# zhoupengwei/tloam

Hardware: AMD Instinct MI355X
Metric: gauss_newton_iters_per_sec (higher is better)
Workload: dtype f64

## Files before the change

tloam_amd/csrc/tl_api.hip:

```cpp
#include "tl_ctx.hpp"

using namespace tl;

extern "C" {

int tloam_abi_version(void) { return TLOAM_ABI_VERSION; }

const char* tloam_status_string(int s) {
  switch (s) {
    case TLOAM_OK: return "ok";
    case TLOAM_E_INVALID: return "invalid argument";
    case TLOAM_E_TOO_FEW_POINTS: return "fewer than 10 points in a feature cloud";
    case TLOAM_E_BAD_POSE: return "predicted pose is not a rigid transform";
    case TLOAM_E_HIP: return "HIP error / no gfx950 device";
    case TLOAM_E_RCCL: return "RCCL error";
    case TLOAM_E_NOT_READY: return "call sequence violated";
    case TLOAM_E_WEIGHT_RANGE: return "GNC weight outside [0,1]";
    default: return "unknown status";
  }
}

void tloam_default_config(tloam_tls_config* c) {
  if (!c) return;
  memset(c, 0, sizeof(*c));
  c->k_corr = 10;
  c->factor_num = 4;
  c->edge_dist_thres = 1.0;
  c->edge_dir_thres = 0.85;
  c->edge_maxnum = 1200;
  c->sphere_dist_thres = 0.5;
  c->sphere_maxnum = 200;
  c->planar_dist_thres = 0.5;
  c->planar_maxnum = 2500;
  c->ground_dist_thres = 0.5;
  c->ground_maxnum = 2000;
  c->max_iterations = 4;
  c->cost_threshold = 5e-9;
  c->gnc_factor = 11.8;
  c->noise_bound = 0.01;
  c->fitness_thres = 0.02;
}

int tloam_create(const tloam_tls_config* cfg, int device_id, tloam_ctx** out) {
  if (!cfg || !out) return TLOAM_E_INVALID;
  *out = nullptr;
  (void)setenv("HIP_FORCE_DEV_KERNARG", "1", 0);
  int ndev = 0;
  if (hipGetDeviceCount(&ndev) != hipSuccess || ndev <= 0 || device_id < 0 || device_id >= ndev) return TLOAM_E_HIP;
  if (hipSetDevice(device_id) != hipSuccess) return TLOAM_E_HIP;
  tloam_ctx* c = new (std::nothrow) tloam_ctx();
  if (!c) return TLOAM_E_INVALID;
  c->cfg = *cfg;
  c->device = device_id;
  if (const char* e = getenv("TLOAM_DEBUG_MAX_SWEEPS")) c->dbg_max_sweeps = atoi(e);
  c->dbg_no_build_reuse = getenv("TLOAM_NO_BUILD_REUSE") != nullptr;
  c->dbg_no_eval_reuse = getenv("TLOAM_NO_EVAL_REUSE") != nullptr;
  c->no_device_loop = getenv("TLOAM_NO_DEVICE_LOOP") != nullptr;
  c->no_persistent_solve = getenv("TLOAM_NO_PERSISTENT_SOLVE") != nullptr;
  c->no_grid_ahead = getenv("TLOAM_NO_GRID_AHEAD") != nullptr;
  c->no_direct_set = getenv("TLOAM_NO_DIRECT_SET") != nullptr;
  c->no_qbin_ride = getenv("TLOAM_NO_QBIN_RIDE") != nullptr;
  if (const char* e = getenv("TLOAM_DEBUG_FAIL_HANDOVER")) c->dbg_fail_handover = atoi(e);
  {
    int cus = 0;
    if (hipDeviceGetAttribute(&cus, hipDeviceAttributeMultiprocessorCount, device_id) != hipSuccess) cus = 0;
    c->device_cus = cus;
  }
  c->fused_large = getenv("TLOAM_FUSED_LARGE") != nullptr;
  if (const char* e = getenv("TLOAM_PLANNED_SWEEPS")) c->dbg_planned_sweeps = atoi(e);
  memset(&c->stats, 0, sizeof(c->stats));
  if (hipStreamCreateWithFlags(&c->stream, hipStreamNonBlocking) != hipSuccess ||
      hipHostMalloc((void**)&c->h_state, sizeof(GnState) * kMirrorSlots, hipHostMallocMapped | hipHostMallocCoherent) != hipSuccess ||
      hipHostMalloc((void**)&c->h_small, sizeof(double) * 4096, hipHostMallocDefault) != hipSuccess) {
    delete c;
    return TLOAM_E_HIP;
  }
  memset(c->h_state, 0, sizeof(GnState) * kMirrorSlots);
  {
    constexpr size_t kBoxBytes = sizeof(double) * ((size_t)kKinds * 64 * 6 + 8);
    const unsigned flags = hipHostMallocMapped | hipHostMallocCoherent;
    if (hipHostMalloc((void**)&c->h_mirror, sizeof(MirrorSlot) * kMirrorSlots, flags) != hipSuccess ||
        ((uintptr_t)c->h_mirror & 63u) != 0 || hipHostGetDevicePointer((void**)&c->h_mirror_dev, c->h_mirror, 0) != hipSuccess ||
        hipHostMalloc((void**)&c->h_bbox, kBoxBytes, flags) != hipSuccess ||
        hipHostGetDevicePointer((void**)&c->h_bbox_dev, c->h_bbox, 0) != hipSuccess ||
        hipHostMalloc((void**)&c->h_fault, sizeof(unsigned) * kFaultWords, flags) != hipSuccess ||
        hipHostGetDevicePointer((void**)&c->h_fault_dev, c->h_fault, 0) != hipSuccess) {
      (void)hipGetLastError();
      tloam_destroy(c);
      return TLOAM_E_HIP;
    }
    memset(c->h_mirror, 0, sizeof(MirrorSlot) * kMirrorSlots);
    memset(c->h_bbox, 0, kBoxBytes);
    memset(c->h_fault, 0, sizeof(unsigned) * kFaultWords);
  }
  if (ensure_common(c) != TLOAM_OK) { tloam_destroy(c); return TLOAM_E_HIP; }
  (void)hipMemsetAsync(c->state.p, 0, sizeof(GnState), c->stream);
  (void)hipMemsetAsync(c->seg_n.p, 0, 8 * sizeof(int), c->stream);
  (void)hipStreamSynchronize(c->stream);
  *out = c;
  return TLOAM_OK;
}

void tloam_destroy(tloam_ctx* c) {
  if (!c) return;
  (void)hipSetDevice(c->device);
  if (c->stream) (void)hipStreamSynchronize(c->stream);
  tlh::comm_release(c);
  c->scan1p_q.release(); c->k3_ticket.release(); c->k3_span.release(); c->iter_span.release(); c->state_scratch.release(); c->blk_cnt.release(); c->row_of_pos.release(); c->fin_tickets.release(); c->fin_rows.release(); c->flagb.release();
  for (auto& e : c->ev_pool) (void)hipEventDestroy(e);
  if (c->frame_selected >= 0) { exchange_clouds(c, *c->frame_store[c->frame_selected]); c->frame_selected = -1; }
  for (int k = 0; k < kKinds; ++k) {
    KindData& K = c->kd[k];
    K.src_aos.release(); K.tgt_aos.release(); K.tx.release(); K.ty.release(); K.tz.release();
    K.c_idx.release(); K.c_buf.release();
// ... 103 lines not shown
```

tloam_amd/csrc/tl_api_match.hip:

```cpp
#include <atomic>
#include <chrono>

#include "tl_ctx.hpp"

using namespace tl;

namespace {
int sync_stream(tloam_ctx* c) {
  HIPC(c, hipStreamSynchronize(c->stream));
  return TLOAM_OK;
}
}

namespace tlh {
int reserve_seg(tloam_ctx* c, int k, size_t n) {
  KindData& K = c->kd[k];
  const size_t cap = round_up(std::max<size_t>(n, 1), kChunk) + kChunk;
  HIPC(c, K.c_idx.reserve(cap));
  if (cap > K.c_stride) {
    const size_t stride = std::max(cap, K.c_stride + K.c_stride / 2);
    HIPC(c, K.c_buf.reserve(stride * kSegStreams));
    K.c_stride = stride;
  }
  K.c_cap = cap - kChunk;
// ... 385 lines not shown
constexpr int kMaxOuterFast = kMirrorSlots;

void outer_params(const tloam_ctx* c, BuildParams* bp, GridView grids[kKinds]) {
  for (int k = 0; k < kKinds; ++k) {
    bp->radius[k] = kind_radius(c->cfg, k);
    bp->maxnum[k] = kind_maxnum(c->cfg, k);
    bp->active[k] = kind_active(c->cfg, k);
    grids[k] = c->kd[k].gv;
  }
  bp->edge_dir_thres = c->cfg.edge_dir_thres;
}
int outer_reserve(tloam_ctx* c, const GridView grids[kKinds]) { return tlh::reserve_query_sort(c, grids); }
}
extern "C++" {
namespace tlh {
int reserve_query_sort(tloam_ctx* c, const GridView grids[kKinds]) {
  const size_t n_slots = (size_t)c->sv.slot_off[kKinds];
  const size_t ntiles = (size_t)build_tile_count(grids, c->sv.slot_off);
  const size_t nt_res = (ntiles + 1 > c->tile_cnt.cap || ntiles + 1 > c->tile_scan.cap) ? 2 * ntiles + 64 : ntiles;
  {
    const size_t before = c->tile_cnt.cap;
    HIPC(c, c->tile_cnt.reserve(nt_res + 1));
    if (c->tile_cnt.cap != before)
      HIPC(c, hipMemsetAsync(c->tile_cnt.p, 0, c->tile_cnt.cap * sizeof(unsigned long long), c->stream));
  }
  HIPC(c, c->tile_scan.reserve(nt_res + 1));
  HIPC(c, c->tile_fill.reserve(std::max<size_t>((size_t)nt_res, (size_t)n_slots + 1))  ); HIPC(c, c->tile_of_slot.reserve(n_slots + 1));
  HIPC(c, c->qrec.reserve(n_slots + 1));
  HIPC(c, c->scan_tmp.reserve(scan_tmp_elems(std::max(nt_res + 1, n_slots + 1))));
  c->scan1p_q_use = !c->no_scan_1p && scan_1p_applies(ntiles + 1, c->device_cus);
  if (c->scan1p_q_use) {
    const size_t before = c->scan1p_q.cap;
    HIPC(c, c->scan1p_q.reserve(scan_1p_ctl_elems(nt_res + 1)));
    if (c->scan1p_q.cap != before) HIPC(c, hipMemsetAsync(c->scan1p_q.p, 0, c->scan1p_q.cap * sizeof(unsigned long long), c->stream));
  }
  return TLOAM_OK;
}
}
}
namespace {
bool prepare_small_path(const tloam_ctx* c) { return one_rank(c) && prepare_small_fits(c->sv); }
bool self_prepare_path(const tloam_ctx* c) { return c->sv.flagb != nullptr && prepare_small_path(c) && solve_small_path(c); }
int enqueue_build(tloam_ctx* c, const BuildParams& bp, const GridView grids[kKinds], bool rebin, const int* gate,
                  const int* refresh_gate = nullptr, bool prepare_in_solve = false, const FinishLargeArgs* ride = nullptr, int iter = 0) {
  const size_t n_slots = (size_t)c->sv.slot_off[kKinds];
  const DirectSet ds{c->direct ? 1 : 0, rebin ? 1 : 0, (ride && !rebin) ? 0 : 1, c->direct ? direct_blk_cnt(c, iter) : nullptr,
                     c->tile_of_slot.p, c->tile_scan.p, c->direct ? c->row_of_pos.p : nullptr};
  if (ride && !rebin) {
    const size_t ntiles = (size_t)build_tile_count(grids, c->sv.slot_off);
    launch_build_finish_large(c->sv, grids, bp, c->state.p, c->tile_scan.p + ntiles, c->qrec.p, *ride, c->stream, c->direct ? &ds : nullptr);
  } else {
    launch_build(c->sv, grids, bp, c->state.p, c->tile_of_slot.p, c->tile_cnt.p, c->tile_scan.p, c->tile_fill.p,
                 c->qrec.p, c->scan_tmp.p, rebin, c->stream, gate, c->scan1p_q_use ? c->scan1p_q.p : nullptr, c->h_fault_dev + kFaultScan1p,
                 c->direct ? &c->cv : nullptr, c->direct ? &ds : nullptr, rebin && c->qbin_rode);
    if (rebin) c->qbin_rode = false;
  }
  if (c->direct) return TLOAM_OK;
  if (prepare_in_solve) return TLOAM_OK;
  if (prepare_small_path(c)) {
    launch_prepare_small(c->sv, c->cv, bp, c->seg_n.p, c->state.p, gate, refresh_gate, c->stream);
    return TLOAM_OK;
  }
  if (one_rank(c)) {
    const int tiles = scan_tiles_only(c->flags.p, c->scan.p, n_slots + 1, c->scan_tmp.p, c->stream, gate);
    if (tiles > 0) {
      launch_compact(c->sv, c->cv, bp, c->seg_n.p, nullptr, 0, 1, c->state.p, c->stream, gate, refresh_gate, c->scan_tmp.p, tiles);
      return TLOAM_OK;
    }
  }
  launch_exclusive_scan_u64(c->flags.p, c->scan.p, n_slots + 1, c->scan_tmp.p, c->stream, gate);
  const double* rank_counts = nullptr;
  if (exchanging(c)) {
    launch_rank_counts(c->sv, c->rank_counts.p, c->rank, c->nranks, c->stream);
    const int rc = allreduce(c, c->rank_counts.p, c->nranks * kKinds);
    if (rc != TLOAM_OK) return rc;
    rank_counts = c->rank_counts.p;
  }
  if (exchanging(c)) HIPC(c, hipMemsetAsync(c->seg_n.p, 0, kKinds * sizeof(int), c->stream));
  launch_compact(c->sv, c->cv, bp, c->seg_n.p, rank_counts, c->rank, c->nranks, c->state.p, c->stream, gate);
  if (refresh_gate) launch_refresh(c->sv, c->cv, c->stream, refresh_gate);
  return TLOAM_OK;
}
int planned_sweeps_for(tloam_ctx* c, int iter) {
  if ((int)c->planned_sweeps.size() < 3 * (iter + 1)) c->planned_sweeps.resize(3 * ((size_t)iter + 1), 0);
  const int* hist = &c->planned_sweeps[3 * (size_t)iter];
  int planned = hist[0] == 0 ? kSolveSweeps
                             : std::min(std::max(std::max(hist[0], hist[1]), std::max(hist[2], 1)), kSolveSweeps);
  if (solve_small_path(c)) planned = kSolveSweeps;
  if (c->dbg_planned_sweeps > 0) planned = std::min(c->dbg_planned_sweeps, kSolveSweeps);
  return planned;
}
WeightParams weight_params(const tloam_ctx* c, double mu, const BuildParams& bp) {
  WeightParams wp;
  wp.th1 = (mu + 1) / mu * c->noise_bound_sq;
  wp.th2 = mu / (mu + 1) * c->noise_bound_sq;
  wp.mu = mu;
  wp.noise_bound_sq = c->noise_bound_sq;
  for (int k = 0; k < kKinds; ++k) wp.active[k] = bp.active[k];
  return wp;
}
size_t total_seg_cap(const tloam_ctx* c) {
  size_t cap = 0;
  for (int k = 0; k < kKinds; ++k) cap += c->kd[k].c_cap;
  return cap;
}
int slot_error(tloam_ctx* c, int incomplete, bool* hand_over_timed_out) {
  if (incomplete == OS_COMM_ERROR) {
// ... 125 lines not shown
    rc = wait_state(c, hm);
    if (rc != TLOAM_OK) return rc;
    if (!c->h_state->incomplete) break;
    if (c->h_state->incomplete == OS_COMM_ERROR) return slot_error(c, OS_COMM_ERROR, nullptr);
    if (attempt > 0 || planned >= kSolveSweeps) return slot_error(c, OS_INCOMPLETE, nullptr);
    rc = enqueue_solve(c, true, kSolveSweeps - planned, &wp);
    if (rc != TLOAM_OK) return rc;
  }
  const GnState& S = *c->h_state;
  rc = harvest_k3_events(c, S.gn_sweeps - sweeps_before);
  if (rc != TLOAM_OK) return rc;
  bool weight_violation = false;
  const bool fin = account_outer(c, iter, S, mu, sweeps_before, &weight_violation);
  if (c->direct) c->w_parity = (iter + 1) & 1;
  if (done) *done = fin ? 1 : 0;
  if (stats) *stats = c->stats;
  return weight_violation ? TLOAM_E_WEIGHT_RANGE : TLOAM_OK;
}

namespace {
struct DeviceLoopPlan {
  int planned[kMaxOuterFast] = {}, solve_start[kMaxOuterFast] = {}, used[kMaxOuterFast] = {};
  double mus[kMaxOuterFast] = {};
  HostMirror hms[kMaxOuterFast];
  bool in_launch_finish = false;
  int enq_end = 0;
  SolveFinish F;
  SolvePrep prep;
};
constexpr int kEnqueueAhead = 2;
int enqueue_iterations_in_launch_mode(tloam_ctx* c, int from, int to, const BuildParams& bp, const GridView grids[kKinds],
                                      DeviceLoopPlan& P) {
  GnState* st = c->state.p;
  for (int iter = from; iter < to; ++iter) {
    int rc = enqueue_build(c, bp, grids, iter == 0, iter == 0 ? nullptr : &st->run_build, nullptr, true);
    if (rc != TLOAM_OK) return rc;
    P.prep.run_build = iter == 0 ? nullptr : &st->run_build;
    P.prep.run_refresh = iter == 0 ? nullptr : &st->run_refresh;
    P.F.first_iter = iter;
    P.planned[iter] = planned_sweeps_for(c, iter);
    P.solve_start[iter] = c->batch_launches;
    rc = enqueue_solve(c, true, P.planned[iter], &P.F.wp[iter], &P.prep, &P.F);
    if (rc != TLOAM_OK) return rc;
  }
  if (to > P.enq_end) P.enq_end = to;
  return TLOAM_OK;
}
int enqueue_outer_iterations(tloam_ctx* c, int first, double mu, const BuildParams& bp, const GridView grids[kKinds],
                             DeviceLoopPlan& P) {
  const int M = c->cfg.max_iterations;
  GnState* st = c->state.p;
  const int* run_build = &st->run_build;
  const int* run_refresh = &st->run_refresh;
  const bool ride = prepare_small_path(c) && finish_small_path(c) && build_finish_small_fits(c->sv);
  const bool ride_large = !ride && one_rank(c) && !finish_small_path(c) && build_finish_large_fits(c->sv);
  const int wblocks_large = finish_wblocks(c);
  if (ride_large) HIPC(c, c->fin_rows.reserve((size_t)4 * 256 * 8));
  bool pending = false;
  bool pending_large = false;
  WeightParams wp_prev;
  OuterCtl ctl_prev{0.0, 0, 0};
  int rc = TLOAM_OK;
  const bool in_solve = self_prepare_path(c);
  SolvePrep prep;
  memset(&prep, 0, sizeof(prep));
  prep.sv = c->sv;
  for (int k = 0; k < kKinds; ++k) prep.maxnum[k] = bp.maxnum[k];
  const bool fin_in_solve = in_solve && finish_small_path(c) && M <= kMaxOuterInLaunch;
  P.in_launch_finish = fin_in_solve;
  if (fin_in_solve) {
    SolveFinish& F = P.F;
    memset(&F, 0, sizeof(F));
    F.enabled = 1;
    F.have_wp = 1;
    F.n_iter = M;
    F.cost_threshold = c->cfg.cost_threshold;
    F.sums16 = c->sums16.p;
    F.iter_span = iter_span_of(c);
    double m = mu;
    for (int iter = first; iter < M; ++iter) {
      P.mus[iter] = m;
      P.hms[iter] = next_mirror(c, iter);
      F.wp[iter] = weight_params(c, m, bp);
      F.hm[iter] = P.hms[iter];
      m = m * exp((double)(iter + 1) * c->cfg.gnc_factor);
    }
    P.prep = prep;
    P.enq_end = first;
    return enqueue_iterations_in_launch_mode(c, first, std::min(M, first + kEnqueueAhead), bp, grids, P);
  }
  for (int iter = first; iter < M; ++iter) {
    if (c->direct) direct_set_parity(c, iter);
    if (iter == 0) {
      rc = enqueue_build(c, bp, grids, true, nullptr, nullptr, in_solve);
      prep.run_build = nullptr;
      prep.run_refresh = nullptr;
    } else if (pending) {
      FinishSmallArgs fin{&c->cv, &wp_prev, c->seg_n.p, c->sums16.p, P.hms[iter - 1], ctl_prev, c->wpart.p, c->k3_ticket.p + 1};
      launch_build_finish_small(c->sv, grids, bp, st, fin, c->stream);
      if (!in_solve) launch_prepare_small(c->sv, c->cv, bp, c->seg_n.p, st, run_build, run_refresh, c->stream);
      prep.run_build = run_build;
      prep.run_refresh = run_refresh;
      pending = false;
    } else if (pending_large) {
      FinishLargeArgs fin{&c->cv, &wp_prev, c->seg_n.p, c->sums16.p, P.hms[iter - 1], ctl_prev, c->fin_rows.p, c->k3_ticket.p + 1,
                          wblocks_large, {}};
      CorrView cv_prev = c->cv;
// ... 576 lines not shown
  HIPC(c, hipEventElapsedTime(&ms, e0, e1));
  (void)hipEventDestroy(e0);
  (void)hipEventDestroy(e1);
  *mean_us = (double)ms * 1e3 / launches;
  return TLOAM_OK;
}

int tloam_time_sharded_sweep(tloam_ctx* c, const double se3[6], int launches, int with_exchange, double* mean_us) {
  if (!c || !se3 || launches < 1 || !mean_us) return TLOAM_E_INVALID;
  HIPC(c, hipSetDevice(c->device));
  if (!c->partials.p) return TLOAM_E_NOT_READY;
  memcpy(c->h_small, se3, sizeof(double) * 6);
  HIPC(c, hipMemcpyAsync(c->se3_dev.p, c->h_small, sizeof(double) * 6, hipMemcpyHostToDevice, c->stream));
  launch_set_eval(c->state.p, c->se3_dev.p, c->stream);
  K3Fuse fuse;
  memset(&fuse, 0, sizeof(fuse));
  fuse.ticket = c->k3_ticket.p;
  fuse.out48 = c->red48.p;
  const bool mbox = with_exchange && c->comm == COMM_MAILBOX && exchanging(c);
  if (mbox) fuse.mb = c->mbox;
  hipEvent_t e0, e1;
  HIPC(c, hipEventCreate(&e0));
  HIPC(c, hipEventCreate(&e1));
  HIPC(c, hipEventRecord(e0, c->stream));
  int rc = TLOAM_OK;
  for (int i = 0; i < launches && rc == TLOAM_OK; ++i) {
    launch_k3_fused(c->cv, c->state.p, c->partials.p, c->k3_grid, c->k3_single, c->k3_wide, true, fuse, c->stream);
    if (mbox) launch_mbox_gather_only(c->red48.p, c->mbox, c->stream);
    else if (with_exchange) rc = allreduce(c, c->red48.p, kReduceBuf);
  }
  HIPC(c, hipEventRecord(e1, c->stream));
  HIPC(c, hipEventSynchronize(e1));
  float ms = 0.f;
  HIPC(c, hipEventElapsedTime(&ms, e0, e1));
  (void)hipEventDestroy(e0);
  (void)hipEventDestroy(e1);
  *mean_us = (double)ms * 1e3 / launches;
  return rc;
}

int tloam_time_build(tloam_ctx* c, int launches, double* mean_us, int64_t* queries) {
  if (!c || launches < 1 || !mean_us) return TLOAM_E_INVALID;
  HIPC(c, hipSetDevice(c->device));
  if (c->active || !c->have_build || !c->qrec.p) return TLOAM_E_NOT_READY;
  BuildParams bp;
  GridView grids[kKinds];
  outer_params(c, &bp, grids);
  hipEvent_t e0, e1;
  HIPC(c, hipEventCreate(&e0));
  HIPC(c, hipEventCreate(&e1));
  HIPC(c, hipEventRecord(e0, c->stream));
  for (int i = 0; i < launches; ++i)
    launch_build(c->sv, grids, bp, c->state.p, c->tile_of_slot.p, c->tile_cnt.p, c->tile_scan.p, c->tile_fill.p, c->qrec.p,
                 c->scan_tmp.p, false, c->stream, nullptr);
  HIPC(c, hipEventRecord(e1, c->stream));
  HIPC(c, hipEventSynchronize(e1));
  float ms = 0.f;
  HIPC(c, hipEventElapsedTime(&ms, e0, e1));
  (void)hipEventDestroy(e0);
  (void)hipEventDestroy(e1);
  *mean_us = (double)ms * 1e3 / launches;
  if (queries) *queries = (int64_t)c->sv.slot_off[kKinds];
  return TLOAM_OK;
}

int tloam_k3_timer(tloam_ctx* c, int reset, double* total_us, int64_t* launches, double* algorithmic_bytes) {
  if (!c) return TLOAM_E_INVALID;
  if (total_us) *total_us = c->k3_total_us;
  if (launches) *launches = c->k3_launches;
  if (algorithmic_bytes) *algorithmic_bytes = c->k3_alg_bytes;
  if (reset) {
    c->k3_total_us = c->k3_all_us = 0.0;
    c->k3_launches = c->k3_all_launches = 0;
  }
  c->k3_timing = true;
  return TLOAM_OK;
}

int tloam_debug_se3(tloam_ctx* c, int n, const double* x, const double* delta, double* out26) {
  if (!c || n < 1 || !x || !delta || !out26) return TLOAM_E_INVALID;
  HIPC(c, hipSetDevice(c->device));
  HIPC(c, c->misc.reserve((size_t)n * 38 + 8));
  double* dx = c->misc.p; double* dd = dx + 6 * (size_t)n; double* dout = dd + 6 * (size_t)n;
  HIPC(c, hipMemcpyAsync(dx, x, sizeof(double) * 6 * n, hipMemcpyHostToDevice, c->stream));
  HIPC(c, hipMemcpyAsync(dd, delta, sizeof(double) * 6 * n, hipMemcpyHostToDevice, c->stream));
  launch_debug_se3(dx, dd, n, dout, c->stream);
  HIPC(c, hipMemcpyAsync(out26, dout, sizeof(double) * 26 * n, hipMemcpyDeviceToHost, c->stream));
  HIPC(c, hipStreamSynchronize(c->stream));
  return TLOAM_OK;
}

int tloam_debug_state(tloam_ctx* c, double* out, int n_doubles) {
  if (!c || !out) return TLOAM_E_INVALID;
  HIPC(c, hipSetDevice(c->device));
  HIPC(c, hipStreamSynchronize(c->stream));
  const size_t bytes = std::min(sizeof(GnState), sizeof(double) * (size_t)n_doubles);
  HIPC(c, hipMemcpy(out, c->state.p, bytes, hipMemcpyDeviceToHost));
  return (int)(sizeof(GnState) / sizeof(double));
}

int tloam_debug_partials(tloam_ctx* c, double* out, int n_doubles) {
  if (!c || !out) return TLOAM_E_INVALID;
  HIPC(c, hipSetDevice(c->device));
  HIPC(c, hipStreamSynchronize(c->stream));
  const size_t n = std::min(c->partials.cap, (size_t)std::max(n_doubles, 0));
  HIPC(c, hipMemcpy(out, c->partials.p, n * sizeof(double), hipMemcpyDeviceToHost));
  return c->k3_grid;
// ... 40 lines not shown
```

tloam_amd/csrc/tl_common.hpp:

```cpp
#pragma once
#include <cstddef>

#include <hip/hip_runtime.h>
#include <stdint.h>

#include "../../include/tloam_hip.h"
#include "tl_se3.hpp"

namespace tl {

constexpr int kKinds = 4;
constexpr int kAccN = 28;
constexpr int kAccStride = 32;
constexpr int kReduceBuf = 48;
constexpr int kChunk = 128;
constexpr int kMaxK = 8;
constexpr int kMaxRanks = 16;

__host__ __device__ inline int res_type_of_kind(int kind) {
  return kind == TLOAM_KIND_EDGE ? TLOAM_RES_LINE : (kind == TLOAM_KIND_SPHERE ? TLOAM_RES_POINT : TLOAM_RES_PLANE);
}

struct GridView {
  const double4* gp;
// ... 197 lines not shown
    int k = 0;
#pragma unroll
    for (int q = 1; q < kKinds; ++q) k += (slot >= fi.slot_off[q]) ? 1 : 0;
    const double* a = fi.src_aos[k] + 3 * (size_t)(slot - fi.slot_off[k]);
    b.sx[slot] = a[0]; b.sy[slot] = a[1]; b.sz[slot] = a[2];
    b.w_src[slot] = 1.0;
  }
  for (int i = block * 256 + (int)threadIdx.x; i < fi.n_tile_cnt; i += nblocks * 256) fi.tile_cnt[i] = 0ull;
  if (block == 0) {
    constexpr int kWords = (int)(sizeof(GnState) / sizeof(double));
    for (int i = threadIdx.x; i < kWords; i += 256) reinterpret_cast<double*>(b.st)[i] = 0.0;
    if (threadIdx.x < 8)
      b.seg_n[threadIdx.x] = (fi.direct && threadIdx.x < kKinds) ? fi.slot_off[threadIdx.x + 1] - fi.slot_off[threadIdx.x] : 0;
    if (threadIdx.x == 0) b.flags[n] = 0ull;
    __syncthreads();
    if (threadIdx.x == 0) {
      GnState* st = b.st;
#pragma unroll
      for (int i = 0; i < 6; ++i) st->x[i] = fi.x[i];
      st->T_cur = se3_exp(st->x);
      st->no_eval_reuse = fi.no_eval_reuse;
      st->prev_planar = __builtin_inf();
      st->run_build = 1;
      arm_solver(*st);
    }
  }
}
#endif
void launch_frame_init(const FrameInit& fi, const FrameInitBufs& b, hipStream_t s);
void launch_bbox_all(const GridSet& gs, double* out , hipStream_t s);
void launch_grid_count_all(const GridSet& gs, unsigned long long* cell_cnt, int* cell_of_pt, int* rank_of_pt,
                           hipStream_t s, const FrameInitHook* frame = nullptr);
void launch_grid_finalize_all(const GridSet& gs, const unsigned long long* cell_scan, int* cell_start,
                              unsigned long long* cell_cnt , hipStream_t s);
int scan_tiles_only(const unsigned long long* in, unsigned long long* out, size_t n, unsigned long long* totals, hipStream_t s,
                    const int* gate = nullptr);
void launch_grid_finalize_scatter_all(const GridSet& gs, const unsigned long long* cell_scan, const unsigned long long* totals,
                                      int tiles, int* cell_start, unsigned long long* cell_cnt, const int* cell_of_pt,
                                      const int* rank_of_pt, double4* gp, hipStream_t s);
void launch_grid_scatter_all(const GridSet& gs, const int* cell_of_pt, const unsigned long long* cell_scan,
                             const int* rank_of_pt, double4* gp, hipStream_t s);
size_t scan_1p_ctl_elems(size_t n);
bool scan_1p_applies(size_t n, int device_cus);
void launch_scan_counts_1p(const unsigned long long* in, unsigned long long* out, size_t n, unsigned long long* ctl, unsigned* fault,
                           hipStream_t s);
void launch_grid_scan_finalize_scatter_1p(const GridSet& gs, unsigned long long* cell_cnt, size_t ncells_plus_1, int* cell_start,
                                          unsigned long long* ctl, unsigned* fault, const int* cell_of_pt, const int* rank_of_pt, double4* gp,
                                          hipStream_t s, const QueryBinRide* qbin = nullptr, const GridView* views = nullptr);

void launch_build(const SlotView& sv, const GridView grids[kKinds], const BuildParams& bp, GnState* st,
                  int* tile_of_slot, unsigned long long* tile_cnt, unsigned long long* tile_scan, int* tile_fill,
                  double4* qrec, unsigned long long* scan_tmp, bool rebin, hipStream_t s, const int* gate = nullptr,
                  unsigned long long* scan1p_ctl = nullptr, unsigned* scan1p_fault = nullptr, const CorrView* direct_cv = nullptr,
                  const DirectSet* ds = nullptr, bool binned = false);
bool direct_set_size(int n_slots);
int build_tile_count(const GridView grids[kKinds], const int slot_off[kKinds + 1]);
void launch_compact(const SlotView& sv, const CorrView& cv, const BuildParams& bp, int* seg_n,
                    const double* rank_counts, int rank, int nranks, GnState* st, hipStream_t s, const int* gate = nullptr,
                    const int* refresh_gate = nullptr, const unsigned long long* totals = nullptr, int tiles = 0);
void launch_rank_counts(const SlotView& sv, double* rank_counts, int rank, int nranks, hipStream_t s);
void launch_refresh(const SlotView& sv, const CorrView& cv, hipStream_t s, const int* gate = nullptr);
bool prepare_small_fits(const SlotView& sv);
void launch_prepare_small(const SlotView& sv, const CorrView& cv, const BuildParams& bp, int* seg_n, GnState* st,
                          const int* run_build, const int* run_refresh, hipStream_t s);
void launch_knn(const GridView& g, const double* qx, const double* qy, const double* qz, int nq,
                double radius, int k, int* out_idx, double* out_d2, int* out_cnt, hipStream_t s);
void launch_fitness(const GridView& g, const double* qx, const double* qy, const double* qz, int nq,
                    double radius, double* partial , int blocks, hipStream_t s);

struct VoxelJob {
  const double *x, *y, *z;
  size_t n, n0;
  double lo[2][3], hi[2][3];
  double voxel[2];
  unsigned long long mask;
};
struct VoxelWork {
  double* min_partial;
  double* vmin;
  unsigned long long *keys, *cnt, *off;
  int *slot_of_pt, *urank, *members, *sorted;
  unsigned long long *leader, *leader_scan;
  unsigned long long* scan_tmp;
  int* overflow;
  unsigned long long* n_out;
  unsigned long long* host_seg;
  unsigned long long host_seq;
  double* out[2][3];
  int use_ticket;
  unsigned* fault;
};
size_t voxel_table_size(size_t n);
int vox_emit_resident_blocks(int device_cus);
void launch_transform_to_soa(const double* aos, size_t n, const double M[16], double* ox, double* oy, double* oz,
                             hipStream_t s);
void launch_transform_to_soa2(const double* aos, size_t n, const double M[16], double* ax, double* ay, double* az,
                              double* bx, double* by, double* bz, hipStream_t s);
struct AssembleArgs {
  const double *ox[2], *oy[2], *oz[2];
  const double* aos[2];
  size_t n_old[2], n_new[2], base[2];
  double M[16];
};
void launch_assemble(const AssembleArgs& A, double* wx, double* wy, double* wz, hipStream_t s);
int transform_ring_max();
void launch_transform_ring(int count, const double* const aos[], const size_t n[], const double* const poses[],
                           double* ax, double* ay, double* az, double* bx, double* by, double* bz, hipStream_t s);
// ... 123 lines not shown
```

tloam_amd/csrc/tl_ctx.hpp:

```cpp
#pragma once

#include <dlfcn.h>
#include <math.h>
#include <stdio.h>
#include <stdlib.h>
#include <string.h>

#include <algorithm>
#include <new>
#include <string>
#include <vector>

#include "tl_common.hpp"


namespace tlh {
using namespace tl;


template <class T>
struct DBuf {
  T* p = nullptr;
  size_t cap = 0;
  hipError_t reserve(size_t n) {
// ... 143 lines not shown
  int dbg_max_sweeps = 0;
  bool dbg_no_build_reuse = false;
  bool dbg_no_eval_reuse = false;
  bool no_device_loop = false;
  bool no_persistent_solve = false;
  bool hand_over_timed_out = false;
  int dbg_fail_handover = 0;
  int device_cus = 0;
  double* h_bbox = nullptr;
  double* h_bbox_dev = nullptr;
  double tgt_box[tl::kKinds][6];
  bool tgt_box_valid[tl::kKinds] = {false, false, false, false};
  double wait_us = 0.0;
  double hs[8] = {0, 0, 0, 0, 0, 0, 0, 0};
  long hs_n = 0;
  double hs_exit = 0.0;
  double hs_entry = 0.0;
  tl::MirrorSlot* h_mirror = nullptr;
  tl::MirrorSlot* h_mirror_dev = nullptr;
  unsigned long long mirror_seq = 0;
  unsigned* h_fault = nullptr;
  unsigned* h_fault_dev = nullptr;
  bool scan1p_retried = false;
  bool vox_ticket = false;
  DBuf<double> src_pack;
  double* h_stage[2] = {nullptr, nullptr};
  double* h_stage_dev[2] = {nullptr, nullptr};
  size_t h_stage_cap[2] = {0, 0};
  hipEvent_t stage_ev[2] = {nullptr, nullptr};
  bool stage_busy[2] = {false, false};
  int stage_next = 0;
  std::vector<tlh::FrameClouds*> frame_store;
  int frame_selected = -1;
  int dbg_planned_sweeps = 0;
  std::vector<int> planned_sweeps;
  bool prebuilt = false;
  int rank = 0, nranks = 1;
  CommMode comm = COMM_NONE;
  bool loopback = false;
  tloam_allreduce_fn cb = nullptr;
  void* cb_user = nullptr;
  void* nccl_comm = nullptr;
  double* mbox_local = nullptr;
  void* mbox_opened[tl::kMaxRanks] = {};
  tl::MboxView mbox{};
  DBuf<unsigned long long> mbox_ctr;
  DBuf<int> k3_ticket;
  DBuf<unsigned long long> k3_span;
  DBuf<unsigned long long> iter_span;
  bool iter_timing = false;
  int fallback_events = 0;
  bool persistent_solve_timed_out = false;
  bool no_qbin_ride = false;
  bool qbin_rode = false;
  bool no_direct_set = false;
  bool direct = false;
  bool set_stale = false;
  int w_parity = 0;
  DBuf<GnState> state_scratch;
  DBuf<int> row_of_pos;
  DBuf<int> fin_tickets;
  DBuf<int> blk_cnt;
  size_t blk_cnt_n = 0;
  bool active = false;
  bool have_build = false;
  double build_x[6] = {0, 0, 0, 0, 0, 0};
  int iter = 0;
  double mu = 1.0, noise_bound_sq = 1e-4;
  double prev_cost[kKinds], cur_cost[kKinds];
  tloam_stats stats;
  bool k3_timing = false;
  std::vector<hipEvent_t> ev_pool;
  size_t ev_used = 0;
  std::vector<int> ev_batch_idx;
  int batch_launches = 0;
  long long k3_seq = 0;
  double k3_total_us = 0.0, k3_all_us = 0.0;
  int64_t k3_launches = 0, k3_all_launches = 0;
  double k3_alg_bytes = 0.0;
  std::string last_error;
};

#define HIPC(ctx, expr)                                                                 \
  do {                                                                                  \
    hipError_t _e = (expr);                                                             \
    if (_e != hipSuccess) {                                                             \
      (ctx)->last_error = std::string(#expr) + ": " + hipGetErrorString(_e);            \
      return TLOAM_E_HIP;                                                               \
    }                                                                                   \
  } while (0)

constexpr int kMirrorSlots = 8;
constexpr int kFaultWords = 16;
constexpr int kFaultScan1p = 0, kFaultVoxEmit = 1;
constexpr size_t kMaxPoints = (size_t)1 << 28;

namespace tlh {
inline double kind_radius(const tloam_tls_config& c, int k) {
  switch (k) {
    case TLOAM_KIND_PLANAR: return c.planar_dist_thres;
    case TLOAM_KIND_GROUND: return c.ground_dist_thres;
    case TLOAM_KIND_EDGE: return c.edge_dist_thres;
    default: return c.sphere_dist_thres;
  }
}
inline int kind_maxnum(const tloam_tls_config& c, int k) {
// ... 41 lines not shown
```

tloam_amd/csrc/tl_nn.hip:

```cpp
#include <string.h>
#include <algorithm>
#include <atomic>

#include "tl_common.hpp"
#include "tl_knn.hpp"
#include "tl_finish.hpp"

namespace tl {

__global__ void k_aos_to_soa(const double* __restrict__ aos, size_t n, double* __restrict__ x,
                             double* __restrict__ y, double* __restrict__ z) {
  size_t i = (size_t)blockIdx.x * blockDim.x + threadIdx.x;
  const size_t stride = (size_t)gridDim.x * blockDim.x;
  for (; i < n; i += stride) {
    x[i] = aos[3 * i];
    y[i] = aos[3 * i + 1];
    z[i] = aos[3 * i + 2];
  }
}
void launch_aos_to_soa(const double* aos, size_t n, double* x, double* y, double* z, hipStream_t s) {
  if (n == 0) return;
  int blocks = (int)((n + 255) / 256);
  if (blocks > 4096) blocks = 4096;
  hipLaunchKernelGGL(k_aos_to_soa, dim3(blocks), dim3(256), 0, s, aos, n, x, y, z);
// ... 815 lines not shown
    else store_raw(A.sv, slot, rec);
  }
  TL_K1_STAMP(7)
  return (rec.flag >> 32) != 0ull;
}

template <int LPQ>
__device__ __forceinline__ void build_sorted_block(const BuildArgs& A, const GnState* __restrict__ st,
                                                   const unsigned long long* __restrict__ n_sorted,
                                                   const double4* __restrict__ qrec, int blk, int2* __restrict__ lds_rows) {
  constexpr int kXcdChunk = 16;
  const int xcd = blk & 7, in_xcd = blk >> 3;
  const int lb0 = ((in_xcd / kXcdChunk) * 8 + xcd) * kXcdChunk + in_xcd % kXcdChunk;
  const int ns = A.identity_n ? A.identity_n : (int)*n_sorted;
  const int nblk = (int)(((long long)ns * LPQ + 63) / 64);
  if (lb0 >= nblk) return;
  const int lb = nblk - 1 - lb0;
  const int t = lb * 64 + threadIdx.x;
  const int i = t / LPQ, sub = t % LPQ;
  if (LPQ != 1 && i >= ns) return;
  if (ns <= 0) return;
  const bool live = i < ns;
  const int qi = live ? i : ns - 1;
  const double4 q = A.identity_n ? double4{A.sv.sx[qi], A.sv.sy[qi], A.sv.sz[qi], __longlong_as_double((long long)qi)} : qrec[qi];
  const int slot = (int)__double_as_longlong(q.w);
  const int kind = slot_kind(A.sv, slot);
  int row_pos = qi;
  if (LPQ == 1 && A.ds.on && A.ds.row_of_pos) {
    if (A.ds.first) {
      if (live) {
        const int t = A.ds.tile_of_slot[slot];
        const unsigned long long s0 = A.ds.tile_scan[t], e0 = A.ds.tile_scan[t + 1];
        if (e0 - s0 > 1ull && e0 - s0 <= (unsigned long long)kDirectBinMax) {
          int rank = 0;
          for (unsigned long long j = s0; j < e0; ++j) rank += ((int)__double_as_longlong(qrec[j].w) < slot) ? 1 : 0;
          row_pos = (int)s0 + rank;
        }
        A.ds.row_of_pos[qi] = row_pos;
      }
    } else {
      row_pos = A.ds.row_of_pos[qi];
    }
  }
  const bool valid = query_one<LPQ>(A, kind, st->T_cur, q, slot, live ? sub : 1, lds_rows, row_pos);
  if (LPQ == 1 && A.ds.on && A.ds.blk_cnt) {
    const bool f = live && valid;
#pragma unroll
    for (int k = 0; k < kKinds; ++k) {
      const int cnt = __popcll(__ballot(f && kind == k));
      if (threadIdx.x == 0) A.ds.blk_cnt[(size_t)lb * kKinds + k] = cnt;
    }
  }
}
template <int LPQ>
__global__ __launch_bounds__(64) void k_build_sorted(BuildArgs A, const GnState* __restrict__ st,
                                                     const unsigned long long* __restrict__ n_sorted,
                                                     const double4* __restrict__ qrec, const int* __restrict__ gate, GnState* st_w) {
  if (gate && *gate == 0) return;
#ifdef TLOAM_K1_PROF
  if (LPQ == 16 && threadIdx.x == 0 && blockIdx.x == 0) g_k1_prof[15] = wall_clock64();
#endif
  __shared__ int2 lds_rows[LPQ == 1 ? 9 * 64 : 1];
  if (LPQ == 1 && A.ds.on && A.ds.set_x_build && blockIdx.x == 0 && threadIdx.x < 6) st_w->x_build[threadIdx.x] = st->x[threadIdx.x];
  build_sorted_block<LPQ>(A, st, n_sorted, qrec, (int)blockIdx.x, lds_rows);
}
__global__ __launch_bounds__(64) void k_build_finish_large(BuildArgs A, GnState* st, const unsigned long long* __restrict__ n_sorted,
                                                           const double4* __restrict__ qrec, const int* __restrict__ seg_n,
                                                           double* __restrict__ sums16, HostMirror hm, OuterCtl ctl, WeightArgs W,
                                                           FinishRideLarge R, FinishDirect D) {
  const int nfin = 4 * R.wblocks;
  if ((int)blockIdx.x < nfin) {
    if (A.ds.on) finish_direct_block(st, seg_n, sums16, hm, ctl, W, D, (int)blockIdx.x);
    else weights_finish_large_ride(st, seg_n, sums16, hm, ctl, W, R, (int)blockIdx.x);
    return;
  }
  if (st->spec_build == 0 || __hip_atomic_load(&st->stop, __ATOMIC_RELAXED, __HIP_MEMORY_SCOPE_AGENT) != 0) return;
  __shared__ int2 lds_rows[9 * 64];
  build_sorted_block<1>(A, st, n_sorted, qrec, (int)blockIdx.x - nfin, lds_rows);
}
__global__ __launch_bounds__(64) void k_finish_direct(GnState* st, const int* __restrict__ seg_n, double* __restrict__ sums16, HostMirror hm,
                                                      OuterCtl ctl, WeightArgs W, FinishDirect D) {
  finish_direct_block(st, seg_n, sums16, hm, ctl, W, D, (int)blockIdx.x);
}
void launch_finish_direct(const FinishLargeArgs& fin, GnState* st, hipStream_t s) {
  WeightArgs W;
  memset(&W, 0, sizeof(W));
  W.cv = *fin.cv;
  W.wp = *fin.wp;
  FinishDirect D{fin.rows, fin.ticket, 4 * fin.wblocks, {fin.w_next[0], fin.w_next[1], fin.w_next[2], fin.w_next[3]}, fin.blk_cnt, fin.nblk, fin.built};
  hipLaunchKernelGGL(k_finish_direct, dim3(4 * fin.wblocks), dim3(64), 0, s, st, fin.seg_n, fin.sums16, fin.hm, fin.ctl, W, D);
}
void launch_grid_scan_finalize_scatter_1p(const GridSet& gs, unsigned long long* cell_cnt, size_t ncells_plus_1, int* cell_start,
                                          unsigned long long* ctl, unsigned* fault, const int* cell_of_pt, const int* rank_of_pt, double4* gp,
                                          hipStream_t s, const QueryBinRide* qbin, const GridView* views) {
  const size_t tiles = (ncells_plus_1 + kTile1p - 1) / kTile1p;
  Scan1p C{ctl, next_scan_epoch(), fault};
  hipLaunchKernelGGL(k_grid_scan_finalize_1p, dim3((unsigned)tiles), dim3(kScanThreads), 0, s, gs, cell_cnt, ncells_plus_1, cell_start, C);
  int blocks = (max_n(gs) + 255) / 256;
  if (blocks > 4096) blocks = 4096;
  if (qbin && views) {
    BuildArgs A;
    memset(&A, 0, sizeof(A));
    A.sv = qbin->sv;
    A.bp = qbin->bp;
    for (int k = 0; k < kKinds; ++k) A.grid[k] = views[k];
    (void)tile_meta(views, qbin->sv.slot_off, &A.tm);
    const int n = qbin->sv.slot_off[kKinds];
    const int rows = std::max(1, std::min(4, ((n + 255) / 256 + blocks - 1) / blocks));
    hipLaunchKernelGGL(k_grid_scatter_qbin, dim3(blocks * (kKinds + rows)), dim3(256), 0, s, gs, cell_of_pt, cell_start, rank_of_pt, gp, A, qbin->st,
                       qbin->tile_of_slot, qbin->rank_in_tile, qbin->tile_cnt, rows);
    return;
  }
  hipLaunchKernelGGL(k_grid_scatter_start_all, dim3(blocks, kKinds), dim3(256), 0, s, gs, cell_of_pt, cell_start, rank_of_pt, gp);
}
void launch_build(const SlotView& sv, const GridView grids[kKinds], const BuildParams& bp, GnState* st,
                  int* tile_of_slot, unsigned long long* tile_cnt, unsigned long long* tile_scan, int* tile_fill,
                  double4* qrec, unsigned long long* scan_tmp, bool rebin, hipStream_t s, const int* gate,
                  unsigned long long* scan1p_ctl, unsigned* scan1p_fault, const CorrView* direct_cv, const DirectSet* ds, bool binned) {
  const int n = sv.slot_off[kKinds];
  if (n <= 0) return;
  BuildArgs A;
  A.sv = sv;
  A.bp = bp;
  memset(&A.ds, 0, sizeof(A.ds));
  memset(&A.cv, 0, sizeof(A.cv));
  if (direct_cv && ds && direct_set_size(n)) { A.ds = *ds; A.cv = *direct_cv; }
  for (int k = 0; k < kKinds; ++k) A.grid[k] = grids[k];
  const int ntiles = tile_meta(grids, sv.slot_off, &A.tm);
  A.identity_n = (n <= kWideLimit) ? n : 0;
  if (rebin && !A.identity_n) {
    if (!binned) hipLaunchKernelGGL(k_query_bin, dim3((n + 255) / 256), dim3(256), 0, s, A, st, tile_of_slot, tile_fill, tile_cnt);
    if (scan1p_ctl) launch_scan_counts_1p(tile_cnt, tile_scan, (size_t)ntiles + 1, scan1p_ctl, scan1p_fault, s);
    else launch_exclusive_scan_u64(tile_cnt, tile_scan, (size_t)ntiles + 1, scan_tmp, s);
    hipLaunchKernelGGL(k_query_scatter, dim3((n + 255) / 256), dim3(256), 0, s, sv, tile_of_slot, tile_scan,
                       tile_fill, qrec);
  }
  auto grid8 = [](long long threads) { return (unsigned)(((threads + 63) / 64 + 127) / 128 * 128); };
  if (n <= kWideLimit)
    hipLaunchKernelGGL(k_build_sorted<16>, dim3(grid8(16LL * n)), dim3(64), 0, s, A, st, tile_scan + ntiles, qrec, gate, st);
  else if (n <= kQuadLimit)
    hipLaunchKernelGGL(k_build_sorted<4>, dim3(grid8(4LL * n)), dim3(64), 0, s, A, st, tile_scan + ntiles, qrec, gate, st);
  else
    hipLaunchKernelGGL(k_build_sorted<1>, dim3(grid8(n)), dim3(64), 0, s, A, st, tile_scan + ntiles, qrec, gate, st);
}
__global__ __launch_bounds__(1024) void k_weights_finish_small(GnState* st, const int* __restrict__ seg_n,
                                                               double* __restrict__ sums16, HostMirror hm, OuterCtl ctl,
                                                               WeightArgs A) {
  weights_finish_small_body(st, seg_n, sums16, hm, ctl, A);
}
void launch_weights_finish_small(const CorrView& cv, const SlotView& sv, const WeightParams& wp, const int* seg_n,
                                 double* sums16, GnState* st, HostMirror hm, OuterCtl ctl, hipStream_t s) {
  WeightArgs A;
  A.cv = cv;
  A.sv = sv;
  A.wp = wp;
  hipLaunchKernelGGL(k_weights_finish_small, dim3(1), dim3(1024), 0, s, st, seg_n, sums16, hm, ctl, A);
}
constexpr int kFinishBlocks = 16;
__global__ __launch_bounds__(64) void k_build_finish_small(BuildArgs A, GnState* st, const int* __restrict__ seg_n,
                                                           double* __restrict__ sums16, HostMirror hm, OuterCtl ctl,
                                                           WeightArgs W, FinishRide R) {
  if (blockIdx.x < kFinishBlocks) {
    weights_finish_small_ride(st, seg_n, sums16, hm, ctl, W, R, (int)blockIdx.x);
    return;
  }
  if (st->spec_build == 0 || __hip_atomic_load(&st->stop, __ATOMIC_RELAXED, __HIP_MEMORY_SCOPE_AGENT) != 0) return;
  constexpr int kXcdChunk = 16;
  const int b = (int)blockIdx.x - kFinishBlocks;
  const int xcd = b & 7, in_xcd = b >> 3;
  const int lb0 = ((in_xcd / kXcdChunk) * 8 + xcd) * kXcdChunk + in_xcd % kXcdChunk;
  const int n = A.identity_n;
  const int nblk = (int)(((long long)n * 16 + 63) / 64);
  if (lb0 >= nblk) return;
  const int t = (nblk - 1 - lb0) * 64 + (int)threadIdx.x;
  const int i = t >> 4, sub = t & 15;
  if (i >= n) return;
  const double4 q = double4{A.sv.sx[i], A.sv.sy[i], A.sv.sz[i], __longlong_as_double((long long)i)};
  query_one<16>(A, slot_kind(A.sv, i), st->T_cur, q, i, sub, nullptr);
}
bool build_finish_small_fits(const SlotView& sv) { return sv.slot_off[kKinds] > 0 && sv.slot_off[kKinds] <= kWideLimit; }
void launch_build_finish_small(const SlotView& sv, const GridView grids[kKinds], const BuildParams& bp, GnState* st,
                               const FinishSmallArgs& fin, hipStream_t s) {
  const int n = sv.slot_off[kKinds];
  BuildArgs A;
  A.sv = sv;
  A.bp = bp;
  for (int k = 0; k < kKinds; ++k) A.grid[k] = grids[k];
  memset(&A.tm, 0, sizeof(A.tm));
  memset(&A.ds, 0, sizeof(A.ds));
  memset(&A.cv, 0, sizeof(A.cv));
  A.identity_n = n;
  WeightArgs W;
  W.cv = *fin.cv;
  W.sv = sv;
  W.wp = *fin.wp;
  const unsigned build_blocks = (unsigned)(((16LL * n + 63) / 64 + 127) / 128 * 128);
// ... 357 lines not shown
```

Baseline: 61520.

## Split multi-lane build kernel into search phase and one-lane-per-query fit phase via LDS

For the multi-lane (LPQ>1) correspondence build kernel, the neighbour search now writes its top-k distances and coordinates to shared memory. After a barrier, one thread per query performs the geometric fit and store, so the fit no longer runs redundantly or divergently across the sub-lanes. Blocks grow to several waves (4 for the quad path, 2 for the wide path) so each block holds enough queries to fill the fit phase. An env flag forces the old single-lane path and disables the small build-finish ride. The change costs extra LDS and a block barrier, and during the fit phase most of the block's threads sit idle.

Result: no change. 61940 (median of 6 runs) (+0.7%).

```diff
diff --git a/tloam_amd/csrc/tl_api.hip b/tloam_amd/csrc/tl_api.hip
--- a/tloam_amd/csrc/tl_api.hip
+++ b/tloam_amd/csrc/tl_api.hip
@@ -60,6 +60,7 @@
   c->no_grid_ahead = getenv("TLOAM_NO_GRID_AHEAD") != nullptr;
   c->no_direct_set = getenv("TLOAM_NO_DIRECT_SET") != nullptr;
   c->no_qbin_ride = getenv("TLOAM_NO_QBIN_RIDE") != nullptr;
+  c->k1_one_lane = getenv("TLOAM_K1_ONE_LANE") != nullptr;
   if (const char* e = getenv("TLOAM_DEBUG_FAIL_HANDOVER")) c->dbg_fail_handover = atoi(e);
   {
     int cus = 0;
diff --git a/tloam_amd/csrc/tl_api_match.hip b/tloam_amd/csrc/tl_api_match.hip
--- a/tloam_amd/csrc/tl_api_match.hip
+++ b/tloam_amd/csrc/tl_api_match.hip
@@ -461,7 +461,7 @@
   } else {
     launch_build(c->sv, grids, bp, c->state.p, c->tile_of_slot.p, c->tile_cnt.p, c->tile_scan.p, c->tile_fill.p,
                  c->qrec.p, c->scan_tmp.p, rebin, c->stream, gate, c->scan1p_q_use ? c->scan1p_q.p : nullptr, c->h_fault_dev + kFaultScan1p,
-                 c->direct ? &c->cv : nullptr, c->direct ? &ds : nullptr, rebin && c->qbin_rode);
+                 c->direct ? &c->cv : nullptr, c->direct ? &ds : nullptr, rebin && c->qbin_rode, c->k1_one_lane);
     if (rebin) c->qbin_rode = false;
   }
   if (c->direct) return TLOAM_OK;
@@ -693,7 +693,7 @@
   GnState* st = c->state.p;
   const int* run_build = &st->run_build;
   const int* run_refresh = &st->run_refresh;
-  const bool ride = prepare_small_path(c) && finish_small_path(c) && build_finish_small_fits(c->sv);
+  const bool ride = prepare_small_path(c) && finish_small_path(c) && build_finish_small_fits(c->sv) && !c->k1_one_lane;
   const bool ride_large = !ride && one_rank(c) && !finish_small_path(c) && build_finish_large_fits(c->sv);
   const int wblocks_large = finish_wblocks(c);
   if (ride_large) HIPC(c, c->fin_rows.reserve((size_t)4 * 256 * 8));
@@ -1376,7 +1376,7 @@
   HIPC(c, hipEventRecord(e0, c->stream));
   for (int i = 0; i < launches; ++i)
     launch_build(c->sv, grids, bp, c->state.p, c->tile_of_slot.p, c->tile_cnt.p, c->tile_scan.p, c->tile_fill.p, c->qrec.p,
-                 c->scan_tmp.p, false, c->stream, nullptr);
+                 c->scan_tmp.p, false, c->stream, nullptr, nullptr, nullptr, nullptr, nullptr, false, c->k1_one_lane);
   HIPC(c, hipEventRecord(e1, c->stream));
   HIPC(c, hipEventSynchronize(e1));
   float ms = 0.f;
diff --git a/tloam_amd/csrc/tl_common.hpp b/tloam_amd/csrc/tl_common.hpp
--- a/tloam_amd/csrc/tl_common.hpp
+++ b/tloam_amd/csrc/tl_common.hpp
@@ -273,7 +273,8 @@
                   int* tile_of_slot, unsigned long long* tile_cnt, unsigned long long* tile_scan, int* tile_fill,
                   double4* qrec, unsigned long long* scan_tmp, bool rebin, hipStream_t s, const int* gate = nullptr,
                   unsigned long long* scan1p_ctl = nullptr, unsigned* scan1p_fault = nullptr, const CorrView* direct_cv = nullptr,
-                  const DirectSet* ds = nullptr, bool binned = false);
+                  const DirectSet* ds = nullptr, bool binned = false,
+                  bool one_lane = false);
 bool direct_set_size(int n_slots);
 int build_tile_count(const GridView grids[kKinds], const int slot_off[kKinds + 1]);
 void launch_compact(const SlotView& sv, const CorrView& cv, const BuildParams& bp, int* seg_n,
diff --git a/tloam_amd/csrc/tl_ctx.hpp b/tloam_amd/csrc/tl_ctx.hpp
--- a/tloam_amd/csrc/tl_ctx.hpp
+++ b/tloam_amd/csrc/tl_ctx.hpp
@@ -219,6 +219,7 @@
   int fallback_events = 0;
   bool persistent_solve_timed_out = false;
   bool no_qbin_ride = false;
+  bool k1_one_lane = false;
   bool qbin_rode = false;
   bool no_direct_set = false;
   bool direct = false;
diff --git a/tloam_amd/csrc/tl_nn.hip b/tloam_amd/csrc/tl_nn.hip
--- a/tloam_amd/csrc/tl_nn.hip
+++ b/tloam_amd/csrc/tl_nn.hip
@@ -891,17 +891,130 @@
     }
   }
 }
+#ifndef TLOAM_K1_FIT_WAVES
+#define TLOAM_K1_FIT_WAVES 4
+#endif
+#ifndef TLOAM_K1_WIDE_FIT_WAVES
+#define TLOAM_K1_WIDE_FIT_WAVES 2
+#endif
 template <int LPQ>
-__global__ __launch_bounds__(64) void k_build_sorted(BuildArgs A, const GnState* __restrict__ st,
-                                                     const unsigned long long* __restrict__ n_sorted,
-                                                     const double4* __restrict__ qrec, const int* __restrict__ gate, GnState* st_w) {
+constexpr int fit_waves() { return LPQ == 1 ? 1 : (LPQ >= 16 ? TLOAM_K1_WIDE_FIT_WAVES : TLOAM_K1_FIT_WAVES); }
+#ifndef TLOAM_K1_WIDE_LPQ
+#define TLOAM_K1_WIDE_LPQ 16
+#endif
+#ifndef TLOAM_K1_QUAD_LPQ
+#define TLOAM_K1_QUAD_LPQ 4
+#endif
+constexpr int kWideLpq = TLOAM_K1_WIDE_LPQ, kQuadLpq = TLOAM_K1_QUAD_LPQ;
+template <int LPQ>
+constexpr int search_threads() { return 64 * fit_waves<LPQ>(); }
+template <int LPQ>
+struct FitLds {
+  static constexpr int Q = 64 * fit_waves<LPQ>() / LPQ;
+  double d[5][Q], x[5][Q], y[5][Q], z[5][Q];
+  int slot[Q];
+  int kind[Q];
+};
+template <int LPQ>
+__device__ __forceinline__ void walk_one(const BuildArgs& A, int kind, const Pose& T, const double4& q, int slot, int sub,
+                                         FitLds<LPQ>& F, int f) {
+  const GridView& g = A.grid[kind];
+  if (!A.bp.active[kind] || g.n <= 0) {
+    if (sub == 0) {
+      store_flag(A.sv, slot, (A.bp.active[kind] && kind == TLOAM_KIND_SPHERE) ? 1ull : 0ull);
+      F.kind[f] = -1;
+    }
+    return;
+  }
+  TL_K1_STAMP(0)
+  const Vec3 pw = act(T, Vec3{q.x, q.y, q.z});
+  const PtsGlobal pts{g.gp};
+  const double radius = A.bp.radius[kind];
+  if (kind == TLOAM_KIND_SPHERE) {
+    TopK<1> tk;
+    NbrXyz<1> c;
+    knn_rows<1, LPQ>(g, pts, pw, sub, tk, nullptr, radius, &c);
+    if (sub == 0) { F.d[0][f] = tk.d[0]; F.x[0][f] = c.x[0]; F.y[0][f] = c.y[0]; F.z[0][f] = c.z[0]; }
+  } else {
+    TopK<5> tk;
+    NbrXyz<5> c;
+    knn_rows<5, LPQ>(g, pts, pw, sub, tk, nullptr, radius, &c);
+    if (sub == 0) {
+#pragma unroll
+      for (int m = 0; m < 5; ++m) { F.d[m][f] = tk.d[m]; F.x[m][f] = c.x[m]; F.y[m][f] = c.y[m]; F.z[m][f] = c.z[m]; }
+    }
+  }
+  if (sub == 0) { F.slot[f] = slot; F.kind[f] = kind; }
+}
+template <int LPQ>
+__device__ __forceinline__ void fit_one(const BuildArgs& A, const FitLds<LPQ>& F, int f) {
+  const int kind = F.kind[f];
+  if (kind < 0) return;
+  RawRec rec;
+  rec.a[0] = rec.a[1] = rec.a[2] = rec.b[0] = rec.b[1] = rec.b[2] = rec.d = 0.0;
+  rec.flag = 0ull;
+  const double radius = A.bp.radius[kind];
+  if (kind == TLOAM_KIND_SPHERE) {
+    TopK<1> tk;
+    tk.d[0] = F.d[0][f];
+    tk.j[0] = 0;
+    finish_sphere_xyz(tk, F.x[0][f], F.y[0][f], F.z[0][f], radius, rec);
+  } else {
+    TopK<5> tk;
+    NbrXyz<5> c;
+#pragma unroll
+    for (int m = 0; m < 5; ++m) { tk.d[m] = F.d[m][f]; tk.j[m] = 0; c.x[m] = F.x[m][f]; c.y[m] = F.y[m][f]; c.z[m] = F.z[m][f]; }
+#ifdef TLOAM_K1_DBG_NOFIT
+    rec.a[0] = tk.d[0] + tk.d[4]; rec.flag = (tk.d[4] < __builtin_inf()) ? ((1ull << 32) | 1ull) : 0ull;
+#else
+    finish_knn5_kept(kind, tk, c, radius, A.bp.edge_dir_thres, rec);
+#endif
+  }
+  TL_K1_STAMP(6)
+  store_raw(A.sv, F.slot[f], rec);
+  TL_K1_STAMP(7)
+}
+template <int LPQ>
+__device__ __forceinline__ void build_sorted_block_fit(const BuildArgs& A, const GnState* __restrict__ st,
+                                                       const unsigned long long* __restrict__ n_sorted,
+                                                       const double4* __restrict__ qrec, int blk, FitLds<LPQ>& F) {
+  constexpr int Q = FitLds<LPQ>::Q;
+  constexpr int kXcdChunk = 16;
+  const int xcd = blk & 7, in_xcd = blk >> 3;
+  const int lb0 = ((in_xcd / kXcdChunk) * 8 + xcd) * kXcdChunk + in_xcd % kXcdChunk;
+  const int ns = A.identity_n ? A.identity_n : (int)*n_sorted;
+  const int nblk = (ns + Q - 1) / Q;
+  if (lb0 >= nblk) return;
+  const int lb = nblk - 1 - lb0;
+  const int f = (int)threadIdx.x / LPQ, sub = (int)threadIdx.x % LPQ;
+  const int i = lb * Q + f;
+  if (i < ns) {
+    const double4 q = A.identity_n ? double4{A.sv.sx[i], A.sv.sy[i], A.sv.sz[i], __longlong_as_double((long long)i)} : qrec[i];
+    const int slot = (int)__double_as_longlong(q.w);
+    walk_one<LPQ>(A, slot_kind(A.sv, slot), st->T_cur, q, slot, sub, F, f);
+  } else if (sub == 0) {
+    F.kind[f] = -1;
+  }
+  __syncthreads();
+  if ((int)threadIdx.x < Q) fit_one<LPQ>(A, F, (int)threadIdx.x);
+}
+template <int LPQ>
+__global__ __launch_bounds__(search_threads<LPQ>()) void k_build_sorted(BuildArgs A, const GnState* __restrict__ st,
+                                                                         const unsigned long long* __restrict__ n_sorted,
+                                                                         const double4* __restrict__ qrec, const int* __restrict__ gate,
+                                                                         GnState* st_w) {
   if (gate && *gate == 0) return;
 #ifdef TLOAM_K1_PROF
   if (LPQ == 16 && threadIdx.x == 0 && blockIdx.x == 0) g_k1_prof[15] = wall_clock64();
 #endif
-  __shared__ int2 lds_rows[LPQ == 1 ? 9 * 64 : 1];
-  if (LPQ == 1 && A.ds.on && A.ds.set_x_build && blockIdx.x == 0 && threadIdx.x < 6) st_w->x_build[threadIdx.x] = st->x[threadIdx.x];
-  build_sorted_block<LPQ>(A, st, n_sorted, qrec, (int)blockIdx.x, lds_rows);
+  if constexpr (LPQ == 1) {
+    __shared__ int2 lds_rows[9 * 64];
+    if (A.ds.on && A.ds.set_x_build && blockIdx.x == 0 && threadIdx.x < 6) st_w->x_build[threadIdx.x] = st->x[threadIdx.x];
+    build_sorted_block<1>(A, st, n_sorted, qrec, (int)blockIdx.x, lds_rows);
+  } else {
+    __shared__ FitLds<LPQ> F;
+    build_sorted_block_fit<LPQ>(A, st, n_sorted, qrec, (int)blockIdx.x, F);
+  }
 }
 __global__ __launch_bounds__(64) void k_build_finish_large(BuildArgs A, GnState* st, const unsigned long long* __restrict__ n_sorted,
                                                            const double4* __restrict__ qrec, const int* __restrict__ seg_n,
@@ -955,7 +1068,8 @@
 void launch_build(const SlotView& sv, const GridView grids[kKinds], const BuildParams& bp, GnState* st,
                   int* tile_of_slot, unsigned long long* tile_cnt, unsigned long long* tile_scan, int* tile_fill,
                   double4* qrec, unsigned long long* scan_tmp, bool rebin, hipStream_t s, const int* gate,
-                  unsigned long long* scan1p_ctl, unsigned* scan1p_fault, const CorrView* direct_cv, const DirectSet* ds, bool binned) {
+                  unsigned long long* scan1p_ctl, unsigned* scan1p_fault, const CorrView* direct_cv, const DirectSet* ds, bool binned,
+                  bool one_lane) {
   const int n = sv.slot_off[kKinds];
   if (n <= 0) return;
   BuildArgs A;
@@ -974,13 +1088,17 @@
     hipLaunchKernelGGL(k_query_scatter, dim3((n + 255) / 256), dim3(256), 0, s, sv, tile_of_slot, tile_scan,
                        tile_fill, qrec);
   }
-  auto grid8 = [](long long threads) { return (unsigned)(((threads + 63) / 64 + 127) / 128 * 128); };
-  if (n <= kWideLimit)
-    hipLaunchKernelGGL(k_build_sorted<16>, dim3(grid8(16LL * n)), dim3(64), 0, s, A, st, tile_scan + ntiles, qrec, gate, st);
-  else if (n <= kQuadLimit)
-    hipLaunchKernelGGL(k_build_sorted<4>, dim3(grid8(4LL * n)), dim3(64), 0, s, A, st, tile_scan + ntiles, qrec, gate, st);
+  auto grid8 = [](long long threads, int per_block) {
+    return (unsigned)(((threads + per_block - 1) / per_block + 127) / 128 * 128);
+  };
+  if (n <= kWideLimit && !one_lane)
+    hipLaunchKernelGGL(k_build_sorted<kWideLpq>, dim3(grid8((long long)kWideLpq * n, search_threads<kWideLpq>())),
+                       dim3(search_threads<kWideLpq>()), 0, s, A, st, tile_scan + ntiles, qrec, gate, st);
+  else if (n <= kQuadLimit && !one_lane)
+    hipLaunchKernelGGL(k_build_sorted<kQuadLpq>, dim3(grid8((long long)kQuadLpq * n, search_threads<kQuadLpq>())),
+                       dim3(search_threads<kQuadLpq>()), 0, s, A, st, tile_scan + ntiles, qrec, gate, st);
   else
-    hipLaunchKernelGGL(k_build_sorted<1>, dim3(grid8(n)), dim3(64), 0, s, A, st, tile_scan + ntiles, qrec, gate, st);
+    hipLaunchKernelGGL(k_build_sorted<1>, dim3(grid8(n, 64)), dim3(64), 0, s, A, st, tile_scan + ntiles, qrec, gate, st);
 }
 __global__ __launch_bounds__(1024) void k_weights_finish_small(GnState* st, const int* __restrict__ seg_n,
                                                                double* __restrict__ sums16, HostMirror hm, OuterCtl ctl,
```
